# Advanced-Vision-and-Learning-Lab/sparse-view-3dgs-pack

Hardware: AMD Instinct MI355X
Metric: train-step views/s (fwd+bwd) @1M Gaussians 1080p (higher is better)
Workload: dtype f32

## Files before the change

### sparse-view-3dgs-pack_amd/csrc/gs_api.hip

```cpp
#include <stdio.h>
#include <stdlib.h>
#include <string.h>
#include <math.h>

#include "gs_common.h"
#include "gs_tilecull.h"
#include "gs_prof.h"

static int check_args(const GsView* v, const GsGaussians* g) {
  if (!v || !g) return GS_E_NULL;
  if (g->P < 0 || v->image_width <= 0 || v->image_height <= 0) return GS_E_SHAPE;
  if (g->P == 0) return GS_OK;
  if (!g->means3D || !g->opacities || !v->viewmatrix || !v->projmatrix || !v->bg) return GS_E_NULL;
  if ((g->shs == nullptr) == (g->colors_precomp == nullptr)) return GS_E_SHAPE;
  const bool has_sr = g->scales != nullptr && g->rotations != nullptr;
  const bool any_sr = g->scales != nullptr || g->rotations != nullptr;
  if ((!has_sr && g->cov3D_precomp == nullptr) || (any_sr && g->cov3D_precomp != nullptr)) return GS_E_SHAPE;
  if (g->shs && (g->M < (v->sh_degree + 1) * (v->sh_degree + 1) || !v->campos)) return GS_E_SHAPE;
  if (v->sh_degree < 0 || v->sh_degree > 3) return GS_E_SHAPE;
  if (g->shs_rest && (!g->shs || g->M < 2)) return GS_E_SHAPE;
  if (v->image_width > 65535 * TILE_X || v->image_height > 65535 * TILE_Y) return GS_E_UNSUPPORTED;
  return GS_OK;
}

static bool reached_marking() {
  static const bool on = [] { const char* e = getenv("GS_REACHED_SPLIT"); return !(e && atoi(e) == 0); }();
  return on;
}
static inline bool step_uses_reached(const GsStepState* st) {
  return st && st->reached_split && !st->rows_override && !st->grad_out[0];
}

static inline void tile_grid(const GsView* v, int& gx, int& gy) {
  gx = (v->image_width + TILE_X - 1) / TILE_X;
  gy = (v->image_height + TILE_Y - 1) / TILE_Y;
}

struct RegionLayout {
  uint32_t* count;
  uint2* bucket;
  uint32_t* point_list;
  uint32_t cap;
  int rg_x, rg_y;
};
static int region_layout(const GsView* v, const GsScratch* sc, RegionLayout& rl) {
// ... 236 lines not shown

  if (!sc->binned) {
    rc = forward_bin_stage(v, sc, gv, iv, bv, P, gx, gy, s);
    if (rc) return rc;
  }
  {
    GS_PROF(ST_RENDER_FWD, s);
    launch_render_fwd_wave(iv.ranges, bv.vals[0], W, H, gx, gy, gv.splat, v->bg, iv.final_T, iv.n_contrib, iv.tile_work,
                           sc->tile_order_hint, sc->tile_depth_limit, iv.tile_stop_depth, &gv.hdr->trunc_failed, out_color,
                           out_invdepth, out_extra, fsgs, v->tile_cull ? 0 : 1, s, reached_marking() ? gv.reached : nullptr,
                           &gv.hdr->pad[HDR_REACHED]);
  }
  if (!sc->defer_tile_order) {
    GS_PROF(ST_TILE_ORDER, s);
    launch_tile_order(iv.tile_work, iv.tile_order, (int)T, sc->tile_order_out, iv.tile_stop_depth, sc->tile_depth_limit_out, gx, gy,
                      gv.hdr, s, sc->tile_depth_limit_slack, sc->status_host, sc->step_tag);
  }
  GS_LAUNCH_CHECK(s, v->debug);
  return GS_OK;
}

int gs_backward(const GsView* v, const GsGaussians* g, const int32_t* radii, const GsScratch* sc,
                int64_t num_rendered, const float* dL_dcolor, const float* dL_dinvdepth, const GsGrads* grads,
                void* workspace, size_t workspace_bytes, void* stream) {
  return gs_backward_x(v, g, radii, sc, num_rendered, dL_dcolor, dL_dinvdepth, nullptr, grads, workspace, workspace_bytes,
                       stream);
}

static int backward_impl(const GsView* v, const GsGaussians* g, const int32_t* radii, const GsScratch* sc,
                         int64_t num_rendered, const float* dL_dcolor, const float* dL_dinvdepth, const float* dL_dextra,
                         int fsgs, const GsGrads* grads, void* workspace, size_t workspace_bytes, void* stream,
// ... 32 lines not shown
  a.P = g->P;
  a.D = v->sh_degree;
  a.M = g->M;
  a.means3D = g->means3D;
  a.radii = radii;
  a.shs = g->shs;
  a.shs_rest = g->shs_rest;
  a.scales = g->scales;
  a.rotations = g->rotations;
  a.opacities = g->opacities;
  a.raw_activations = g->raw_activations;
  a.skip_uninstanced = 0;
  a.tiles_touched = gv.tiles_touched;
  a.reached = nullptr;
  a.reached_flag = nullptr;
  a.colors_precomp = g->colors_precomp;
  a.scale_modifier = v->scale_modifier;
  a.cov3D = g->cov3D_precomp ? g->cov3D_precomp : gv.cov3D;
  a.viewmatrix = v->viewmatrix;
  a.projmatrix = v->projmatrix;
  a.campos = v->campos;
  a.focal_y = v->image_height / (2.0f * v->tanfovy);
  a.focal_x = v->image_width / (2.0f * v->tanfovx);
  a.tan_fovx = v->tanfovx;
  a.tan_fovy = v->tanfovy;
  a.antialiasing = v->antialiasing;
  a.has_invdepth = depth_mode;
  a.has_extra = g->extra_channel != nullptr;
  a.extra_raw = a.extra_gain = nullptr;
  a.gain_partials = nullptr;
// ... 88 lines not shown
  }
  if (num_rendered > 0 && !given_rows) {
    {
      GS_PROF(ST_RENDER_BWD, s);
      launch_render_bwd_wave(iv.ranges, bv.vals[0], W, H, gx, gy, gv.splat, v->bg, iv.final_T, iv.n_contrib, iv.tile_work,
                             iv.tile_order, dL_dcolor, dL_dinvdepth, dL_dextra, rows, fsgs, s);
    }
    GS_LAUNCH_CHECK(s, v->debug);
  }
  PreprocessBwdArgs a = preprocess_bwd_args(v, g, radii, gv, fsgs ? 2 : (dL_dinvdepth != nullptr ? 1 : 0), rows, recs, grads);
  a.skip_uninstanced = (v->tile_cull || (step && step->phase == 2)) ? 1 : 0;
  a.clean_rows = rows_clean != 0;
  if (step_uses_reached(step)) {
    a.reached = gv.reached;
    a.reached_flag = &gv.hdr->pad[HDR_REACHED];
  }
  if (step && step->extra) {
    float* gp = reinterpret_cast<float*>((char*)workspace + gs_align((size_t)P * GR_ROW_BYTES) + gs_align((size_t)P * GC_REC_BYTES));
    a.extra_raw = step->extra;
    a.extra_gain = step->gain;
    a.gain_partials = gp;
    sa.gain_partials = gp;
  }
  {
    GS_PROF(ST_CHAIN, s);
    launch_chain(a, step ? gv.hdr : nullptr, s);
  }
  if (step) {
    GS_PROF(ST_BWD_STEP, s);
    sa.hdr = gv.hdr;
// ... 407 lines not shown
  hdr->pad[0] = gs_status_check(t, hdr->num_rendered, hdr->overflow, hdr->trunc_failed);
}

int gs_forward_tile_order(const GsView* v, const GsScratch* sc, void* stream) {
  if (!v || !sc || !sc->geom || !sc->img) return GS_E_NULL;
  const int W = v->image_width, H = v->image_height;
  if (W <= 0 || H <= 0) return GS_E_SHAPE;
  int gx, gy;
  tile_grid(v, gx, gy);
  const size_t T = (size_t)gx * gy, N = (size_t)W * H;
  if (sc->img_bytes < img_bytes(N, T) || sc->geom_bytes < sizeof(GeomHeader)) return GS_E_SCRATCH;
  hipStream_t s = (hipStream_t)stream;
  ImgView iv = img_view(sc->img, N, T);
  GS_PROF(ST_TILE_ORDER, s);
  launch_tile_order(iv.tile_work, iv.tile_order, (int)T, sc->tile_order_out, iv.tile_stop_depth, sc->tile_depth_limit_out, gx, gy,
                    (const GeomHeader*)sc->geom, s, sc->tile_depth_limit_slack, sc->status_host, sc->step_tag);
  GS_LAUNCH_CHECK(s, v->debug);
  return GS_OK;
}

int gs_forward_status(const GsScratch* sc, uint32_t* out, void* stream) {
  if (!sc || !sc->geom || !out) return GS_E_NULL;
  if (sc->geom_bytes < sizeof(GeomHeader)) return GS_E_SCRATCH;
  hipStream_t s = (hipStream_t)stream;
  size_t bytes = 16;
  if (sc->step_tag) {
    (void)hipGetLastError();
    hipLaunchKernelGGL(status_tag_kernel, dim3(1), dim3(1), 0, s, (GeomHeader*)sc->geom, sc->step_tag);
    GS_LAUNCH_CHECK(s, 0);
    bytes = 48;
  }
// ... 96 lines not shown
```

### sparse-view-3dgs-pack_amd/csrc/gs_backward_math.h

```cpp
#pragma once
#include "gs_common.h"
#include "gs_math.h"

struct ShRegsB {
  float f[48];
  __host__ __device__ __forceinline__ V3 operator()(int k) const { return {f[3 * k], f[3 * k + 1], f[3 * k + 2]}; }
};

#define SH_LDS_ROW 19
struct ShSink {
  float* p;
  bool basis_only;
  float* rest = nullptr;
  __host__ __device__ __forceinline__ void rgb(V3 g) const {
    if (basis_only) {
      p[16] = g.x;
      p[17] = g.y;
      p[18] = g.z;
    }
  }
  __host__ __device__ __forceinline__ void set(int k, float basis, V3 g) const {
    if (basis_only) {
      p[k] = basis;
    } else {
// ... 210 lines not shown
}


struct GeomBack {
  V3 dmean;
  float dmean2D_x, dmean2D_y;
  float dcov[6];
  float dop, dextra;
  V3 dcolor;
  V3 dscale;
  float dq[4];
};
GS_DEV void chain_from_row(const PreprocessBwdArgs& a, int idx, const gs_row_t* row, float* rec) {
  const double2* gr = reinterpret_cast<const double2*>(row);
  const double2 g0 = gr[0], g1 = gr[1], g2 = gr[2], g3 = gr[3], g4 = gr[4], g5 = gr[5];
  const V3 mean = {a.means3D[3 * idx], a.means3D[3 * idx + 1], a.means3D[3 * idx + 2]};
  SymD Sg;
  RotD R = {};
  D3 s = {0.0, 0.0, 0.0};
  V4 rq = {1.f, 0.f, 0.f, 0.f};
  if (a.scales) {
    const V3 scl = load_scales(a.scales, idx, a.raw_activations);
    rq = load_rotation(a.rotations, idx, a.raw_activations);
    const double mod = a.scale_modifier;
    s = {mod * scl.x, mod * scl.y, mod * scl.z};
    R = quat_to_Rd(rq);
    Sg = sigma_from_scale_rot(s, R);
  } else {
    const float2* cv = reinterpret_cast<const float2*>(a.cov3D + 6 * (size_t)idx);
    const float2 v0 = cv[0], v1 = cv[1], v2 = cv[2];
// ... 8 lines not shown
    const float* vm = a.viewmatrix;
    const float zc = vm[2] * mean.x + vm[6] * mean.y + vm[10] * mean.z + vm[14];
    const float gd = (float)g4.y;
    dmean = dmean + V3{(vm[2] - vm[3] * zc) * gd, (vm[6] - vm[7] * zc) * gd, (vm[10] - vm[11] * zc) * gd};
  }
  float c[7] = {0.f, 0.f, 0.f, 0.f, 0.f, 0.f, 0.f};
  if (a.scales) {
    V3 dscale;
    cov3d_backward(cb.G, s, R, rq, dscale, c + 3);
    c[0] = dscale.x; c[1] = dscale.y; c[2] = dscale.z;
  } else {
    c[0] = (float)cb.G.xx; c[1] = (float)(2.0 * cb.G.xy); c[2] = (float)(2.0 * cb.G.xz);
    c[3] = (float)cb.G.yy; c[4] = (float)(2.0 * cb.G.yz); c[5] = (float)cb.G.zz;
  }
  float4* o = reinterpret_cast<float4*>(rec);
  o[0] = make_float4((float)g0.x, (float)g0.y, dmean.x, dmean.y);
  o[1] = make_float4(dmean.z, cb.dop, c[0], c[1]);
  o[2] = make_float4(c[2], c[3], c[4], c[5]);
  o[3] = make_float4(c[6], (float)g3.x, (float)g3.y, (float)g4.x);
  o[4] = make_float4((float)g5.x, 0.f, 0.f, 0.f);
}

GS_DEV void geometry_backward(const PreprocessBwdArgs& a, int idx, GeomBack& o) {
  const float4* rc = reinterpret_cast<const float4*>(a.grad_recs + (size_t)idx * GC_STRIDE);
  const float4 r0 = rc[0], r1 = rc[1], r2 = rc[2], r3 = rc[3];
  o.dmean2D_x = r0.x;
  o.dmean2D_y = r0.y;
  o.dop = r1.y;
  o.dcolor = {r3.y, r3.z, r3.w};
  o.dextra = a.has_extra ? a.grad_recs[(size_t)idx * GC_STRIDE + GC_EXTRA] : 0.f;
  const V3 mean = {a.means3D[3 * idx], a.means3D[3 * idx + 1], a.means3D[3 * idx + 2]};
  o.dmean = V3{r0.z, r0.w, r1.x} + projection_backward(mean, a.projmatrix, o.dmean2D_x, o.dmean2D_y);
  o.dscale = {0.f, 0.f, 0.f};
  o.dq[0] = o.dq[1] = o.dq[2] = o.dq[3] = 0.f;
  o.dcov[0] = o.dcov[1] = o.dcov[2] = o.dcov[3] = o.dcov[4] = o.dcov[5] = 0.f;
// ... 54 lines not shown
```

### sparse-view-3dgs-pack_amd/csrc/gs_common.h

```cpp
#pragma once
#include <hip/hip_runtime.h>
#include <stdint.h>

#include "../../include/gsplat.h"

#define GS_BLOCK 256
#define TILE_X GS_TILE_X
#define TILE_Y GS_TILE_Y

struct GeomHeader {
  uint32_t num_rendered;
  uint32_t overflow;
  uint32_t trunc_failed;
  uint32_t zero;
  uint32_t P;
  uint32_t sort_n;
  uint32_t n_ordered;
  uint32_t region_mode;
  uint32_t step_tag;
  uint32_t pad[55];
};
#define HDR_SIDE_CURSOR 1
#define HDR_LIMITED 2
#define HDR_REACHED 3
static_assert(sizeof(GeomHeader) == 256, "header is one 256-B block");

struct __attribute__((aligned(64))) Splat {
  float x, y;
  float depth;
  float invdepth;
  float cxx, cxy, cyy;
  float opacity;
  float r, g, b;
  float extra;
  uint32_t rect_min;
  uint32_t rect_max;
  uint32_t tiles;
  uint32_t clamped;
};
// ... 34 lines not shown
  b.vals[1] = (uint32_t*)p; p += gs_align(4 * cap);
  b.hist = (uint32_t*)p; p += gs_align(4 * hist_n);
  b.scan_tmp = (uint32_t*)p; p += gs_align(4 * RS_RADIX_MAX);
  return b;
}

struct GeomView {
  GeomHeader* hdr;
  Splat* splat;
  float* cov3D;
  uint32_t* tiles_touched;
  uint32_t* block_sums;
  uint32_t* sorted_sums;
  uint32_t* depth_keys;
  SortBufs gsort;
  uint8_t* reached;
};
static inline __host__ __device__ size_t geom_bytes(size_t P) {
  size_t nb = (P + GS_BLOCK - 1) / GS_BLOCK;
  return sizeof(GeomHeader) + gs_align(64 * P) + gs_align(24 * P) + 2 * gs_align(4 * P) + 2 * gs_align(4 * (nb + 1)) +
         sort_bytes(P) + gs_align(P);
}
static inline __host__ __device__ GeomView geom_view(void* buf, size_t P) {
  char* p = (char*)buf;
  size_t nb = (P + GS_BLOCK - 1) / GS_BLOCK;
  GeomView g;
  g.hdr = (GeomHeader*)p; p += sizeof(GeomHeader);
  g.splat = (Splat*)p; p += gs_align(64 * P);
  g.cov3D = (float*)p; p += gs_align(24 * P);
  g.tiles_touched = (uint32_t*)p; p += gs_align(4 * P);
  g.block_sums = (uint32_t*)p; p += gs_align(4 * (nb + 1));
  g.sorted_sums = (uint32_t*)p; p += gs_align(4 * (nb + 1));
  g.depth_keys = (uint32_t*)p; p += gs_align(4 * P);
  g.gsort = sort_view(p, P); p += sort_bytes(P);
  g.reached = (uint8_t*)p;
  return g;
}

#define RG_COUNT_STRIDE 32
struct ImgView {
  float* final_T;
  uint32_t* n_contrib;
  uint2* ranges;
  uint32_t* tile_work;
  uint32_t* tile_order;
  float* tile_stop_depth;
  uint32_t* region_count;
};
static inline __host__ __device__ size_t img_bytes(size_t N, size_t T) {
// ... 141 lines not shown
int launch_region_bin(const GeomView& g, const uint32_t* region_count, const uint2* region_bucket, uint32_t region_cap, int rg_x,
                      int rg_y, int grid_x, int grid_y, const float* tile_depth_limit, uint2* ranges, uint32_t* point_list,
                      int64_t capacity, hipStream_t s);
int launch_export_keys_region(const uint2* ranges, const uint32_t* point_list, const Splat* splat, int T, uint64_t* keys_sorted,
                              hipStream_t s);


int launch_render_fwd_wave(const uint2* ranges, const uint32_t* point_list, int W, int H, int grid_x, int grid_y,
                           const Splat* splat, const float* bg, float* final_T, uint32_t* n_contrib, uint32_t* tile_work,
                           const uint32_t* order_hint, const float* depth_limit, float* stop_depth, uint32_t* trunc_failed,
                           float* out_color, float* out_invdepth, float* out_extra, int fsgs, int cull, hipStream_t s,
                           uint8_t* reached = nullptr, uint32_t* reached_flag = nullptr);
int launch_export_stop_depth(const float* stop_depth, float* out, int grid_x, int grid_y, hipStream_t s);
int launch_tile_order(const uint32_t* tile_work, uint32_t* tile_order, int T, uint32_t* order_out, const float* stop_depth,
                      float* limit_out, int grid_x, int grid_y, const GeomHeader* hdr, hipStream_t s,
                      const float* slack_dev = nullptr, uint32_t* status_host = nullptr, const uint32_t* step_tag = nullptr);
int launch_zero_rows(gs_row_t* rows, size_t P, const uint32_t* tiles_touched, hipStream_t s);
int launch_render_bwd_wave(const uint2* ranges, const uint32_t* point_list, int W, int H, int grid_x, int grid_y,
                           const Splat* splat, const float* bg, const float* final_T, const uint32_t* n_contrib,
                           const uint32_t* tile_work, const uint32_t* tile_order, const float* dL_dpix,
                           const float* dL_dinvdepth, const float* dL_dextra, gs_row_t* grad_rows, int fsgs, hipStream_t s);

int launch_depth_fwd(const uint2* ranges, const uint32_t* point_list, int W, int H, int grid_x, int grid_y, const Splat* splat,
                     float* final_T, uint32_t* n_contrib, uint32_t* tile_work, float* stop_depth, float* out_depth,
                     float* out_alpha, int cull, hipStream_t s);
int launch_depth_bwd(const uint2* ranges, const uint32_t* point_list, int W, int H, int grid_x, int grid_y, const Splat* splat,
                     const float* final_T, const uint32_t* n_contrib, const uint32_t* tile_work, const uint32_t* tile_order,
                     const float* dL_ddepth, const float* dL_dalpha, gs_row_t* grad_rows, int grad_flags, hipStream_t s);
struct DepthPointArgs {
  int P;
  const float* means3D;
// ... 43 lines not shown
  float focal_x, focal_y, tan_fovx, tan_fovy;
  int antialiasing;
  int has_invdepth;
  int has_extra;
  const float* extra_raw;
  const float* extra_gain;
  float* gain_partials;
  int raw_activations;
  int skip_uninstanced;
  const gs_row_t* grad_rows;
  float* grad_recs;
  int clean_rows;
  const uint32_t* tiles_touched;
  const uint8_t* reached;
  const uint32_t* reached_flag;
  const Splat* splat;
  GsGrads out;
};
static inline __device__ bool gs_use_reached(const PreprocessBwdArgs& a) {
  return a.reached != nullptr && a.reached_flag[0] != 0u;
}
static inline __device__ bool gs_instanced(const PreprocessBwdArgs& a, bool use_reached, int idx) {
  return use_reached ? a.reached[idx] != 0 : a.tiles_touched[idx] != 0u;
}
int launch_chain(const PreprocessBwdArgs& a, const GeomHeader* hdr, hipStream_t s);
int launch_preprocess_bwd(const PreprocessBwdArgs& a, hipStream_t s, float* dsh_rest_out = nullptr);
struct StepArgs {
  GsStepState st;
  float lr_bc1[6];
  float inv_sqrt_bc2[5];
// ... 8 lines not shown
```

### sparse-view-3dgs-pack_amd/csrc/gs_preprocess.hip

```cpp
#include "gs_common.h"
#include "gs_tilecull.h"
#include "gs_math.h"

template <typename SH>
GS_DEV V3 color_from_sh(int deg, V3 pos, V3 campos, const SH& sh, uint32_t& clamped) {
  V3 dir = pos - campos;
  dir = dir / length3(dir);
  V3 result = SH_C0 * sh(0);
  if (deg > 0) {
    float x = dir.x, y = dir.y, z = dir.z;
    result = result - SH_C1 * y * sh(1) + SH_C1 * z * sh(2) - SH_C1 * x * sh(3);
    if (deg > 1) {
      float xx = x * x, yy = y * y, zz = z * z;
      float xy = x * y, yz = y * z, xz = x * z;
      result = result + SH_C2_0 * xy * sh(4) + SH_C2_1 * yz * sh(5) + SH_C2_2 * (2.0f * zz - xx - yy) * sh(6) +
               SH_C2_3 * xz * sh(7) + SH_C2_4 * (xx - yy) * sh(8);
      if (deg > 2) {
        result = result + SH_C3_0 * y * (3.0f * xx - yy) * sh(9) + SH_C3_1 * xy * z * sh(10) +
                 SH_C3_2 * y * (4.0f * zz - xx - yy) * sh(11) + SH_C3_3 * z * (2.0f * zz - 3.0f * xx - 3.0f * yy) * sh(12) +
                 SH_C3_4 * x * (4.0f * zz - xx - yy) * sh(13) + SH_C3_5 * z * (xx - yy) * sh(14) +
                 SH_C3_6 * x * (xx - 3.0f * yy) * sh(15);
      }
    }
  }
// ... 82 lines not shown
  float op_in = a.opacities[lidx];
  V3 p_orig = {a.means3D[3 * (size_t)lidx], a.means3D[3 * (size_t)lidx + 1], a.means3D[3 * (size_t)lidx + 2]};
  V3 sc_in = {sc_p[0], sc_p[1], sc_p[2]};
  V4 rq_in = {rq_p[0], rq_p[1], rq_p[2], rq_p[3]};
  if (lds_floats) {
    const float* src = a.tile_depth_limit + (GS_LIMIT_TILES_IN_LDS ? 0 : T);
    for (int i = threadIdx.x; i < lds_floats; i += GS_BLOCK) s_limit[i] = src[i];
    __syncthreads();
  }
  asm volatile("" : "+v"(op_in), "+v"(sc_in.x), "+v"(sc_in.y), "+v"(sc_in.z), "+v"(rq_in.x), "+v"(rq_in.y), "+v"(rq_in.z),
               "+v"(rq_in.w));
  const GsLdsFloatPtr lds_seg = (GsLdsFloatPtr)s_limit + (GS_LIMIT_TILES_IN_LDS ? T : 0);
  if (idx == 0) {
    g.hdr->pad[HDR_LIMITED] = a.tile_depth_limit ? 1u : 0u;
    g.hdr->pad[HDR_REACHED] = 0u;
  }
  const int segs_x = (int)depth_limit_segs_x((uint32_t)a.grid_x);
  auto region_bound = [&](int rx, int ry) {
    float bound = -__builtin_inff();
#pragma unroll
    for (int k = 0; k < RG_TILES; k++) {
      const int ty = min(ry * RG_TILES + k, a.grid_y - 1);
      const float v = lds_floats ? lds_seg[ty * segs_x + rx] : a.tile_depth_limit[(size_t)T + ty * segs_x + rx];
      bound = fmaxf(bound, v);
    }
    return bound;
  };
  Splat sp;
  sp.x = sp.y = sp.depth = sp.invdepth = 0.f;
  sp.cxx = sp.cxy = sp.cyy = sp.opacity = 0.f;
// ... 427 lines not shown
```

### sparse-view-3dgs-pack_amd/csrc/gs_preprocess_bwd.hip

```cpp
#include "gs_common.h"
#include "gs_math.h"
#include "gs_backward_math.h"

#define CHAIN_PER_WAVE 256
__global__ void __launch_bounds__(64, 3) chain_kernel(PreprocessBwdArgs a, const GeomHeader* hdr) {
  __shared__ int s_list[CHAIN_PER_WAVE];
  const int lane = threadIdx.x;
  const int base = blockIdx.x * CHAIN_PER_WAVE;
  bool has[CHAIN_PER_WAVE / 64];
  const bool use_reached = gs_use_reached(a);
  const bool list_reached = use_reached && !a.gain_partials;
#pragma unroll
  for (int k = 0; k < CHAIN_PER_WAVE / 64; k++) {
    const int idx = base + k * 64 + lane;
    has[k] = idx < a.P && a.radii[idx] > 0 && !(a.skip_uninstanced && !gs_instanced(a, list_reached, idx));
  }
  int n = 0;
#pragma unroll
  for (int k = 0; k < CHAIN_PER_WAVE / 64; k++) {
    const unsigned long long m = __ballot(has[k]);
    if (has[k]) s_list[n + __popcll(m & ((1ull << lane) - 1ull))] = base + k * 64 + lane;
    n += __popcll(m);
  }
  __syncthreads();
  const bool failed = hdr && (hdr->overflow | hdr->trunc_failed) != 0u;
  float gc = 1.0f, dgain = 0.f;
  bool gain_free = false;
  if (a.gain_partials) {
    const float gain = *a.extra_gain;
    gc = clamp_gain(gain);
    gain_free = gain >= 0.1f && gain <= 10.0f;
  }
  for (int j = lane; j < n; j += 64) {
    const int idx = s_list[j];
    if (use_reached && !list_reached && a.reached[idx] == 0) continue;
    gs_row_t* row = const_cast<gs_row_t*>(a.grad_rows) + (size_t)idx * GR_STRIDE;
    float* rec = a.grad_recs + (size_t)idx * GC_STRIDE;
    if (!failed) {
      chain_from_row(a, idx, row, rec);
      if (a.gain_partials) {
        const float dextra = rec[GC_EXTRA];
        if (gain_free) dgain += dextra * (1.0f / (1.0f + expf(-a.extra_raw[idx])));
        rec[GC_EXTRA] = dextra * gc;
      }
    }
    if (a.clean_rows) {
      float4* w = reinterpret_cast<float4*>(row);
      w[0] = w[1] = w[2] = w[3] = w[4] = w[5] = make_float4(0.f, 0.f, 0.f, 0.f);
    }
  }
  if (a.gain_partials) {
#pragma unroll
    for (int off = 32; off >= 1; off >>= 1) dgain += __shfl_down(dgain, off, 64);
    if (lane == 0) a.gain_partials[blockIdx.x] = dgain;
  }
}
int launch_chain(const PreprocessBwdArgs& a, const GeomHeader* hdr, hipStream_t s) {
  hipLaunchKernelGGL(chain_kernel, dim3((a.P + CHAIN_PER_WAVE - 1) / CHAIN_PER_WAVE), dim3(64), 0, s, a, hdr);
  return 0;
}

template <int N, typename G>
__device__ __forceinline__ void grad_block(float* __restrict__ out, int first, int cnt, const G& grad) {
// ... 503 lines not shown
```

### sparse-view-3dgs-pack_amd/csrc/gs_render_fwd_wave.hip

```cpp
#include "gs_blend.h"
#include "gs_common.h"
#include "gs_tilecull.h"

#define WB 64

template <bool HAS_EXTRA, bool FSGS, bool CULL>
__global__ void __launch_bounds__(64) render_fwd_wave_kernel(const uint2* __restrict__ ranges,
                                                             const uint32_t* __restrict__ point_list, int W, int H,
                                                             int grid_x, const Splat* __restrict__ splat,
                                                             const float* __restrict__ bg, float* __restrict__ final_T,
                                                             uint32_t* __restrict__ n_contrib,
                                                             uint32_t* __restrict__ tile_work,
                                                             const uint32_t* __restrict__ order_hint,
                                                             const float* __restrict__ depth_limit,
                                                             float* __restrict__ stop_depth,
                                                             uint32_t* __restrict__ trunc_failed,
                                                             float* __restrict__ out_color,
                                                             float* __restrict__ out_invdepth,
                                                             float* __restrict__ out_extra,
                                                             uint8_t* __restrict__ reached,
                                                             uint32_t* __restrict__ reached_flag) {
  __shared__ float4 s_a[WB];
  __shared__ float4 s_c[WB];
  __shared__ float4 s_k[WB];
// ... 155 lines not shown
  if (fsgs) {
    if (cull) GS_FWD_WAVE(false, true, true); else GS_FWD_WAVE(false, true, false);
  } else if (out_extra) {
    if (cull) GS_FWD_WAVE(true, false, true); else GS_FWD_WAVE(true, false, false);
  } else {
    if (cull) GS_FWD_WAVE(false, false, true); else GS_FWD_WAVE(false, false, false);
  }
#undef GS_FWD_WAVE
  return 0;
}

#define TO_THREADS 1024
#define TO_BUCKETS 2048
__device__ __forceinline__ void stop_depth_bound_item(const float* __restrict__ stop, float* __restrict__ out, int grid_x,
                                                      int grid_y, int i, float slack = 1.0f);
__global__ void __launch_bounds__(TO_THREADS) tile_order_kernel(const uint32_t* __restrict__ tile_work,
                                                                uint32_t* __restrict__ tile_order, int T, int per_band,
                                                                uint32_t* __restrict__ order_out,
                                                                const float* __restrict__ stop_depth,
                                                                float* __restrict__ limit_out, int grid_x, int grid_y,
                                                                const GeomHeader* __restrict__ hdr,
                                                                const float* __restrict__ slack_dev,
                                                                uint32_t* status_host, const uint32_t* step_tag) {
  if (status_host && blockIdx.x == 0 && threadIdx.x == 0) {
    const uint32_t nr = hdr->num_rendered, ov = hdr->overflow, tf = hdr->trunc_failed;
    volatile uint32_t* out = status_host;
    out[0] = nr; out[1] = ov; out[2] = tf; out[3] = hdr->zero;
    if (step_tag) {
      const uint32_t t = *step_tag;
      out[9] = gs_status_check(t, nr, ov, tf);
      __threadfence_system();
      out[8] = t;
    }
    __threadfence_system();
  }
  if (hdr->overflow) order_out = nullptr;
  if (blockIdx.x >= 8) {
    const int i = (int)(blockIdx.x - 8) * TO_THREADS + (int)threadIdx.x;
    if (!hdr->overflow && i < (int)depth_limit_floats((uint32_t)grid_x, (uint32_t)grid_y))
      stop_depth_bound_item(stop_depth, limit_out, grid_x, grid_y, i, slack_dev ? fmaxf(*slack_dev, 1.0f) : 1.0f);
    return;
  }
  __shared__ uint32_t s_cnt[TO_BUCKETS];
  __shared__ uint32_t s_part[TO_THREADS / 64];
  __shared__ uint32_t s_max;
  const int tid = threadIdx.x;
  const int band = blockIdx.x;
  const int t_lo = band * per_band, t_hi = min(T, t_lo + per_band);
  uint32_t m = 0;
  for (int t = t_lo + tid; t < t_hi; t += TO_THREADS) m = max(m, tile_work[t]);
#pragma unroll
// ... 58 lines not shown
}
__global__ void __launch_bounds__(256) stop_depth_bounds_kernel(const float* __restrict__ stop, float* __restrict__ out,
                                                                int grid_x, int grid_y) {
  const int i = blockIdx.x * 256 + threadIdx.x;
  if (i < (int)depth_limit_floats((uint32_t)grid_x, (uint32_t)grid_y)) stop_depth_bound_item(stop, out, grid_x, grid_y, i);
}

int launch_export_stop_depth(const float* stop_depth, float* out, int grid_x, int grid_y, hipStream_t s) {
  const int n = (int)depth_limit_floats((uint32_t)grid_x, (uint32_t)grid_y);
  hipLaunchKernelGGL(stop_depth_bounds_kernel, dim3((n + 255) / 256), dim3(256), 0, s, stop_depth, out, grid_x, grid_y);
  return 0;
}

int launch_tile_order(const uint32_t* tile_work, uint32_t* tile_order, int T, uint32_t* order_out, const float* stop_depth,
                      float* limit_out, int grid_x, int grid_y, const GeomHeader* hdr, hipStream_t s, const float* slack_dev,
                      uint32_t* status_host, const uint32_t* step_tag) {
  const int extra = limit_out ? ((int)depth_limit_floats((uint32_t)grid_x, (uint32_t)grid_y) + TO_THREADS - 1) / TO_THREADS : 0;
  hipLaunchKernelGGL(tile_order_kernel, dim3(8 + extra), dim3(TO_THREADS), 0, s, tile_work, tile_order, T, (T + 7) / 8, order_out,
                     stop_depth, limit_out, grid_x, grid_y, hdr, slack_dev, status_host, step_tag);
  return 0;
}
```

### sparse-view-3dgs-pack_amd/gsplat_amd/raster.py

```python
import ctypes as C
import os

import torch

from .capi import GsGaussians, GsGrads, GsScratch, GsView

NUM_CHANNELS = 3
_DEPTH_ONLY = 2


def _ptr(t):
    if t is None or t.numel() == 0:
        return None
    return t.data_ptr()


def _prep(t, device):
    if t is None or t.numel() == 0:
        return None
    if t.dtype != torch.float32:
        t = t.float()
    if t.device != device:
        t = t.to(device)
    return t.contiguous()
# ... 326 lines not shown
        self.api.raw("region_coop")(int(bool(on)))

    scratch_fill = None
    output_fill = None
    KEYED_LIMITS = os.environ.get("GS_KEYED_LIMITS", "1") != "0"
    STATUS_IN_RENDER = True

    def _side_stream(self, device):
        side = self._side_streams.get(device.index)
        if side is None:
            side = self._side_streams[device.index] = torch.cuda.Stream(device=device)
        return side
    TWO_PHASE = os.environ.get("GS_TWO_PHASE_STEP", "1") != "0"
    TWO_PHASE_MIN_P = 100_000
    REACHED_SPLIT = os.environ.get("GS_REACHED_SPLIT", "1") != "0"

    def _two_phase(self, step, P):
        return self.TWO_PHASE and P >= self.TWO_PHASE_MIN_P and not step.grad_out[0]

    def _arms_side_launch(self, step, P):
        return self._two_phase(step, P) and not step.rows_override

    def launch_uninstanced_early(self):
        f = self._last
        if f is None or f.step is None or f.done is not None:
            return False
        f.done = self._launch_uninstanced(f.geom.device, f.view, f.g, f.radii, self._scratch(f.geom, f.img), f.step)
        return True

    def _structs(self, device, bg, means3D, sh, colors_precomp, opacities, scales, rotations, cov3D_precomp, viewmatrix,
                 projmatrix, campos, tanfovx, tanfovy, H, W, scale_modifier, degree, antialiasing, debug, extra=None, raw=False,
                 extra_gain=None, sh_rest=None):
        keep = []
        view = self._view(keep, device, bg, viewmatrix, projmatrix, campos, tanfovx, tanfovy, H, W, scale_modifier, degree,
                          False, antialiasing, debug)
        g = self._gauss(keep, device, means3D, sh, colors_precomp, opacities, scales, rotations, cov3D_precomp, extra, raw=raw,
                        extra_gain=extra_gain, sh_rest=sh_rest)
        return view, g, keep

    def _launch_uninstanced(self, device, view, g, radii, s, step):
        main = torch.cuda.current_stream(device)
        side = self._side_stream(device)
        side.wait_stream(main)
        step.reached_split = int(self.REACHED_SPLIT)
        self.api.call("step_uninstanced", C.byref(view), C.byref(g), radii.contiguous().data_ptr(), C.byref(s),
                      C.byref(step), C.c_void_p(side.cuda_stream))
        done = torch.cuda.Event()
        done.record(side)
        self.two_phase_launches += 1
        return done

    def rasterize_gaussians(self, bg, means3D, colors_precomp, opacities, scales, rotations, scale_modifier,
                            cov3D_precomp, viewmatrix, projmatrix, tanfovx, tanfovy, image_height, image_width,
                            sh, degree, campos, prefiltered, antialiasing, debug, extra=None, fsgs=False, extra_gain=None):
        if fsgs and (extra is not None or antialiasing):
            raise RuntimeError("the FSGS rasterizer generation has neither anti-aliasing nor a 4th channel")
        if means3D.ndim != 2 or means3D.shape[1] != 3:
            raise RuntimeError("means3D must have dimensions (num_points, 3)")
        self._check_device(means3D)
# ... 393 lines not shown
        return z

    def _backward_step_fsgs(self, step, view, g, radii, geom, binning, img, P, W, H, R, dL_dout_color, dL_ddepth, dL_dalpha):
        device = radii.device
        if step.phase != 0 or step.phase1_done:
            raise RuntimeError("the two-phase step (side launch of gs_step_uninstanced) is closed to the FSGS rasterizer "
                               "generation")
        if step.extra:
            raise RuntimeError("the FSGS rasterizer generation has no 4th channel to step")
        _, _, _, wsb = self.scratch_bytes(P, W, H, R)
        ws = self._rows_workspace(step, device, wsb)
        s = self._scratch(geom, img, binning, self._capacity_for(binning, P, W, H, R))
        last = self._last
        if last is not None:
            last.step = last.radii = last.img = last.done = None
        step.reached_split = int(self.REACHED_SPLIT)
        dL_ddepth, dL_dalpha = _prep(dL_ddepth, device), _prep(dL_dalpha, device)
        zeros = self._zero_image(device, H, W) if dL_ddepth is None or dL_dalpha is None else None
        try:
            self.api.call("backward_step_fsgs", C.byref(view), C.byref(g), radii.data_ptr(), C.byref(s), int(R),
                          dL_dout_color.data_ptr(), (dL_ddepth if dL_ddepth is not None else zeros).data_ptr(),
                          (dL_dalpha if dL_dalpha is not None else zeros).data_ptr(), C.byref(step), _ptr(ws), ws.numel(),
                          self._stream(device))
        except Exception:
            self.rows_epoch += 1
            raise
        if step.rows_clean:
            self._rows_ws[(device.index, wsb)][1] = True
        return (None,) * 8

    def _backward_step(self, step, f, view, g, radii, geom, binning, img, P, W, H, R, dL_dout_color, dL_dout_invdepth,
                       dL_dout_extra, fsgs=False):
        if fsgs:
            return self._backward_step_fsgs(step, view, g, radii, geom, binning, img, P, W, H, R, dL_dout_color,
                                            dL_dout_invdepth, dL_dout_extra)
        device = radii.device
        _, _, _, wsb = self.scratch_bytes(P, W, H, R)
        ws = self._rows_workspace(step, device, wsb)
        s = self._scratch(geom, img, binning, self._capacity_for(binning, P, W, H, R))
        done, last = None, self._last
        if last is not None:
            if last is f and last.step is step:
                done = last.done
            last.step = last.radii = last.img = last.done = None
        if done is None:
            step.reached_split = int(self.REACHED_SPLIT)
        if self._two_phase(step, P):
            if done is None:
                done = self._launch_uninstanced(device, view, g, radii, s, step)
            self._uninst_done = done
            step.phase = 2
            step.phase1_done = done.cuda_event
        try:
            if dL_dout_extra is not None:
                self.api.call("backward_step_x", C.byref(view), C.byref(g), radii.data_ptr(), C.byref(s), int(R),
                              dL_dout_color.data_ptr(), _ptr(dL_dout_invdepth), dL_dout_extra.data_ptr(), C.byref(step),
                              _ptr(ws), ws.numel(), self._stream(device))
            else:
                self.api.call("backward_step", C.byref(view), C.byref(g), radii.data_ptr(), C.byref(s), int(R),
                              dL_dout_color.data_ptr(), _ptr(dL_dout_invdepth), C.byref(step), _ptr(ws), ws.numel(),
                              self._stream(device))
# ... 124 lines not shown
        P = int(means3D.shape[0])
        present = torch.zeros((P,), dtype=torch.bool, device=device)
        if P != 0:
            m, vm, pm = (_prep(x, device) for x in (means3D, viewmatrix, projmatrix))
            self.api.call("mark_visible", P, m.data_ptr(), vm.data_ptr(), pm.data_ptr(), present.data_ptr(),
                          self._stream(device))
        return present

    def export_reached(self, P, geom):
        gb = self.scratch_bytes(P, 16, 16, 0)[0]
        off = gb - ((P + 255) // 256) * 256
        if geom.device.type == "cuda":
            torch.cuda.current_stream(geom.device).synchronize()
        return geom[off:off + P].clone()

    def export_state(self, P, W, H, R, geom, binning, img):
        device = geom.device
        cap = self._capacity_for(binning, P, W, H, R)
        s = self._scratch(geom, img, binning, cap)
        f32 = dict(dtype=torch.float32, device=device)
        T = ((W + 15) // 16) * ((H + 15) // 16)
        out = dict(
            depths=torch.zeros((P,), **f32), means2D=torch.zeros((P, 2), **f32), cov3D=torch.zeros((P, 6), **f32),
            conic_opacity=torch.zeros((P, 4), **f32), rgb=torch.zeros((P, 3), **f32),
            clamped=torch.zeros((P, 3), dtype=torch.uint8, device=device),
            tiles_touched=torch.zeros((P,), dtype=torch.int32, device=device),
            point_offsets=torch.zeros((P,), dtype=torch.int32, device=device),
            keys_sorted=torch.zeros((R,), dtype=torch.int64, device=device),
            point_list=torch.zeros((R,), dtype=torch.int32, device=device),
            final_T=torch.zeros((H, W), **f32), n_contrib=torch.zeros((H, W), dtype=torch.int32, device=device),
# ... 18 lines not shown
```

Baseline: 1261.

## Build compacted reached-Gaussian list in tile-order kernel and drive chain backward from it

Extra workgroups appended to the tile-order kernel compact the per-Gaussian reached flags into per-segment index lists with counts. The backward chain kernel then walks this compact list instead of scanning all P Gaussians with radii, instanced and reached checks, so it should launch less idle work when only a fraction were reached. In exchange the geometry scratch grows by about 4 bytes per Gaussian, the tile-order kernel does more work, and every chain wave runs a prefix scan over segment counts. It also pins the rec-store values in registers with empty asm statements.

```diff
diff --git a/sparse-view-3dgs-pack_amd/csrc/gs_api.hip b/sparse-view-3dgs-pack_amd/csrc/gs_api.hip
--- a/sparse-view-3dgs-pack_amd/csrc/gs_api.hip
+++ b/sparse-view-3dgs-pack_amd/csrc/gs_api.hip
@@ -28,7 +28,14 @@
   return on;
 }
 static inline bool step_uses_reached(const GsStepState* st) {
-  return st && st->reached_split && !st->rows_override && !st->grad_out[0];
+  return st && (st->reached_split & 1) && !st->rows_override && !st->grad_out[0];
+}
+static bool reached_listing() {
+  static const bool on = [] { const char* e = getenv("GS_REACHED_LIST"); return !(e && atoi(e) == 0); }();
+  return on && reached_marking();
+}
+static inline bool step_uses_reached_list(const GsStepState* st) {
+  return step_uses_reached(st) && !(st->reached_split & 2) && !st->extra && reached_listing();
 }
 
 static inline void tile_grid(const GsView* v, int& gx, int& gy) {
@@ -295,7 +302,8 @@
   if (!sc->defer_tile_order) {
     GS_PROF(ST_TILE_ORDER, s);
     launch_tile_order(iv.tile_work, iv.tile_order, (int)T, sc->tile_order_out, iv.tile_stop_depth, sc->tile_depth_limit_out, gx, gy,
-                      gv.hdr, s, sc->tile_depth_limit_slack, sc->status_host, sc->step_tag);
+                      gv.hdr, s, sc->tile_depth_limit_slack, sc->status_host, sc->step_tag, reached_listing() ? sc->geom : nullptr,
+                      sc->geom_bytes, P);
   }
   GS_LAUNCH_CHECK(s, v->debug);
   return GS_OK;
@@ -358,6 +366,7 @@
   a.tiles_touched = gv.tiles_touched;
   a.reached = nullptr;
   a.reached_flag = nullptr;
+  a.reached_list = a.reached_counts = a.reached_list_flag = nullptr;
   a.colors_precomp = g->colors_precomp;
   a.scale_modifier = v->scale_modifier;
   a.cov3D = g->cov3D_precomp ? g->cov3D_precomp : gv.cov3D;
@@ -476,6 +485,11 @@
   if (step_uses_reached(step)) {
     a.reached = gv.reached;
     a.reached_flag = &gv.hdr->pad[HDR_REACHED];
+  }
+  if (step_uses_reached_list(step) && sc->geom_bytes >= geom_bytes((size_t)P)) {
+    a.reached_list = gv.reached_list;
+    a.reached_counts = gv.reached_counts;
+    a.reached_list_flag = &gv.hdr->pad[HDR_REACHED_LIST];
   }
   if (step && step->extra) {
     float* gp = reinterpret_cast<float*>((char*)workspace + gs_align((size_t)P * GR_ROW_BYTES) + gs_align((size_t)P * GC_REC_BYTES));
@@ -913,7 +927,8 @@
   ImgView iv = img_view(sc->img, N, T);
   GS_PROF(ST_TILE_ORDER, s);
   launch_tile_order(iv.tile_work, iv.tile_order, (int)T, sc->tile_order_out, iv.tile_stop_depth, sc->tile_depth_limit_out, gx, gy,
-                    (const GeomHeader*)sc->geom, s, sc->tile_depth_limit_slack, sc->status_host, sc->step_tag);
+                    (const GeomHeader*)sc->geom, s, sc->tile_depth_limit_slack, sc->status_host, sc->step_tag,
+                    reached_listing() ? sc->geom : nullptr, sc->geom_bytes, -1);
   GS_LAUNCH_CHECK(s, v->debug);
   return GS_OK;
 }
diff --git a/sparse-view-3dgs-pack_amd/csrc/gs_backward_math.h b/sparse-view-3dgs-pack_amd/csrc/gs_backward_math.h
--- a/sparse-view-3dgs-pack_amd/csrc/gs_backward_math.h
+++ b/sparse-view-3dgs-pack_amd/csrc/gs_backward_math.h
@@ -248,6 +248,8 @@
 GS_DEV void chain_from_row(const PreprocessBwdArgs& a, int idx, const gs_row_t* row, float* rec) {
   const double2* gr = reinterpret_cast<const double2*>(row);
   const double2 g0 = gr[0], g1 = gr[1], g2 = gr[2], g3 = gr[3], g4 = gr[4], g5 = gr[5];
+  float p_mx = (float)g0.x, p_my = (float)g0.y, p_r = (float)g3.x, p_g = (float)g3.y, p_b = (float)g4.x, p_x = (float)g5.x;
+  asm volatile("" : "+v"(p_mx), "+v"(p_my), "+v"(p_r), "+v"(p_g), "+v"(p_b), "+v"(p_x));
   const V3 mean = {a.means3D[3 * idx], a.means3D[3 * idx + 1], a.means3D[3 * idx + 2]};
   SymD Sg;
   RotD R = {};
@@ -286,11 +288,11 @@
     c[3] = (float)cb.G.yy; c[4] = (float)(2.0 * cb.G.yz); c[5] = (float)cb.G.zz;
   }
   float4* o = reinterpret_cast<float4*>(rec);
-  o[0] = make_float4((float)g0.x, (float)g0.y, dmean.x, dmean.y);
+  o[0] = make_float4(p_mx, p_my, dmean.x, dmean.y);
   o[1] = make_float4(dmean.z, cb.dop, c[0], c[1]);
   o[2] = make_float4(c[2], c[3], c[4], c[5]);
-  o[3] = make_float4(c[6], (float)g3.x, (float)g3.y, (float)g4.x);
-  o[4] = make_float4((float)g5.x, 0.f, 0.f, 0.f);
+  o[3] = make_float4(c[6], p_r, p_g, p_b);
+  o[4] = make_float4(p_x, 0.f, 0.f, 0.f);
 }
 
 GS_DEV void geometry_backward(const PreprocessBwdArgs& a, int idx, GeomBack& o) {
diff --git a/sparse-view-3dgs-pack_amd/csrc/gs_common.h b/sparse-view-3dgs-pack_amd/csrc/gs_common.h
--- a/sparse-view-3dgs-pack_amd/csrc/gs_common.h
+++ b/sparse-view-3dgs-pack_amd/csrc/gs_common.h
@@ -23,6 +23,7 @@
 #define HDR_SIDE_CURSOR 1
 #define HDR_LIMITED 2
 #define HDR_REACHED 3
+#define HDR_REACHED_LIST 4
 static_assert(sizeof(GeomHeader) == 256, "header is one 256-B block");
 
 struct __attribute__((aligned(64))) Splat {
@@ -87,12 +88,16 @@
   uint32_t* sorted_sums;
   uint32_t* depth_keys;
   SortBufs gsort;
+  uint32_t* reached_list;
+  uint32_t* reached_counts;
   uint8_t* reached;
 };
+#define RL_SEG 65536
+static inline __host__ __device__ size_t reached_list_segments(size_t P) { return (P + RL_SEG - 1) / RL_SEG; }
 static inline __host__ __device__ size_t geom_bytes(size_t P) {
   size_t nb = (P + GS_BLOCK - 1) / GS_BLOCK;
   return sizeof(GeomHeader) + gs_align(64 * P) + gs_align(24 * P) + 2 * gs_align(4 * P) + 2 * gs_align(4 * (nb + 1)) +
-         sort_bytes(P) + gs_align(P);
+         sort_bytes(P) + gs_align(4 * P) + gs_align(4 * reached_list_segments(P)) + gs_align(P);
 }
 static inline __host__ __device__ GeomView geom_view(void* buf, size_t P) {
   char* p = (char*)buf;
@@ -106,6 +111,8 @@
   g.sorted_sums = (uint32_t*)p; p += gs_align(4 * (nb + 1));
   g.depth_keys = (uint32_t*)p; p += gs_align(4 * P);
   g.gsort = sort_view(p, P); p += sort_bytes(P);
+  g.reached_list = (uint32_t*)p; p += gs_align(4 * P);
+  g.reached_counts = (uint32_t*)p; p += gs_align(4 * reached_list_segments(P));
   g.reached = (uint8_t*)p;
   return g;
 }
@@ -277,7 +284,8 @@
 int launch_export_stop_depth(const float* stop_depth, float* out, int grid_x, int grid_y, hipStream_t s);
 int launch_tile_order(const uint32_t* tile_work, uint32_t* tile_order, int T, uint32_t* order_out, const float* stop_depth,
                       float* limit_out, int grid_x, int grid_y, const GeomHeader* hdr, hipStream_t s,
-                      const float* slack_dev = nullptr, uint32_t* status_host = nullptr, const uint32_t* step_tag = nullptr);
+                      const float* slack_dev = nullptr, uint32_t* status_host = nullptr, const uint32_t* step_tag = nullptr,
+                      void* list_geom = nullptr, size_t list_geom_bytes = 0, int64_t list_P = -1);
 int launch_zero_rows(gs_row_t* rows, size_t P, const uint32_t* tiles_touched, hipStream_t s);
 int launch_render_bwd_wave(const uint2* ranges, const uint32_t* point_list, int W, int H, int grid_x, int grid_y,
                            const Splat* splat, const float* bg, const float* final_T, const uint32_t* n_contrib,
@@ -351,6 +359,9 @@
   const uint32_t* tiles_touched;
   const uint8_t* reached;
   const uint32_t* reached_flag;
+  const uint32_t* reached_list;
+  const uint32_t* reached_counts;
+  const uint32_t* reached_list_flag;
   const Splat* splat;
   GsGrads out;
 };
diff --git a/sparse-view-3dgs-pack_amd/csrc/gs_preprocess.hip b/sparse-view-3dgs-pack_amd/csrc/gs_preprocess.hip
--- a/sparse-view-3dgs-pack_amd/csrc/gs_preprocess.hip
+++ b/sparse-view-3dgs-pack_amd/csrc/gs_preprocess.hip
@@ -120,6 +120,7 @@
   if (idx == 0) {
     g.hdr->pad[HDR_LIMITED] = a.tile_depth_limit ? 1u : 0u;
     g.hdr->pad[HDR_REACHED] = 0u;
+    g.hdr->pad[HDR_REACHED_LIST] = 0u;
   }
   const int segs_x = (int)depth_limit_segs_x((uint32_t)a.grid_x);
   auto region_bound = [&](int rx, int ry) {
diff --git a/sparse-view-3dgs-pack_amd/csrc/gs_preprocess_bwd.hip b/sparse-view-3dgs-pack_amd/csrc/gs_preprocess_bwd.hip
--- a/sparse-view-3dgs-pack_amd/csrc/gs_preprocess_bwd.hip
+++ b/sparse-view-3dgs-pack_amd/csrc/gs_preprocess_bwd.hip
@@ -3,26 +3,64 @@
 #include "gs_backward_math.h"
 
 #define CHAIN_PER_WAVE 256
+__device__ __forceinline__ int chain_list_entry(const PreprocessBwdArgs& a, uint32_t* s_incl, uint32_t e0, uint32_t& total) {
+  const int lane = threadIdx.x;
+  const uint32_t nseg = (uint32_t)reached_list_segments((size_t)a.P);
+  const uint32_t e = e0 + (uint32_t)lane;
+  uint32_t carry = 0u, seg = 0u, off = 0u;
+  bool found = false;
+  for (uint32_t c = 0; c < nseg; c += 64u) {
+    uint32_t incl = (c + lane < nseg) ? a.reached_counts[c + lane] : 0u;
+#pragma unroll
+    for (int o = 1; o < 64; o <<= 1) {
+      const uint32_t up = (uint32_t)__shfl_up((int)incl, o, 64);
+      if (lane >= o) incl += up;
+    }
+    incl += carry;
+    s_incl[lane] = incl;
+    __syncthreads();
+    const uint32_t after = s_incl[63];
+    if (!found && e < after) {
+      int lo = 0;
+#pragma unroll
+      for (int step = 32; step >= 1; step >>= 1)
+        if (s_incl[lo + step - 1] <= e) lo += step;
+      seg = c + (uint32_t)lo;
+      off = e - (lo ? s_incl[lo - 1] : carry);
+      found = true;
+    }
+    carry = after;
+    __syncthreads();
+  }
+  total = carry;
+  const size_t slot = (size_t)seg * RL_SEG + off;
+  if (!found || slot >= (size_t)a.P) return -1;
+  const uint32_t idx = a.reached_list[slot];
+  return (idx < (uint32_t)a.P && a.radii[idx] > 0) ? (int)idx : -1;
+}
 __global__ void __launch_bounds__(64, 3) chain_kernel(PreprocessBwdArgs a, const GeomHeader* hdr) {
   __shared__ int s_list[CHAIN_PER_WAVE];
   const int lane = threadIdx.x;
   const int base = blockIdx.x * CHAIN_PER_WAVE;
   bool has[CHAIN_PER_WAVE / 64];
   const bool use_reached = gs_use_reached(a);
+  const bool list_mode = a.reached_list && use_reached && a.skip_uninstanced && !a.gain_partials && a.reached_list_flag[0] != 0u;
   const bool list_reached = use_reached && !a.gain_partials;
-#pragma unroll
-  for (int k = 0; k < CHAIN_PER_WAVE / 64; k++) {
-    const int idx = base + k * 64 + lane;
-    has[k] = idx < a.P && a.radii[idx] > 0 && !(a.skip_uninstanced && !gs_instanced(a, list_reached, idx));
-  }
   int n = 0;
-#pragma unroll
-  for (int k = 0; k < CHAIN_PER_WAVE / 64; k++) {
-    const unsigned long long m = __ballot(has[k]);
-    if (has[k]) s_list[n + __popcll(m & ((1ull << lane) - 1ull))] = base + k * 64 + lane;
-    n += __popcll(m);
-  }
-  __syncthreads();
+  if (!list_mode) {
+#pragma unroll
+    for (int k = 0; k < CHAIN_PER_WAVE / 64; k++) {
+      const int idx = base + k * 64 + lane;
+      has[k] = idx < a.P && a.radii[idx] > 0 && !(a.skip_uninstanced && !gs_instanced(a, list_reached, idx));
+    }
+#pragma unroll
+    for (int k = 0; k < CHAIN_PER_WAVE / 64; k++) {
+      const unsigned long long m = __ballot(has[k]);
+      if (has[k]) s_list[n + __popcll(m & ((1ull << lane) - 1ull))] = base + k * 64 + lane;
+      n += __popcll(m);
+    }
+    __syncthreads();
+  }
   const bool failed = hdr && (hdr->overflow | hdr->trunc_failed) != 0u;
   float gc = 1.0f, dgain = 0.f;
   bool gain_free = false;
@@ -31,22 +69,36 @@
     gc = clamp_gain(gain);
     gain_free = gain >= 0.1f && gain <= 10.0f;
   }
-  for (int j = lane; j < n; j += 64) {
-    const int idx = s_list[j];
-    if (use_reached && !list_reached && a.reached[idx] == 0) continue;
-    gs_row_t* row = const_cast<gs_row_t*>(a.grad_rows) + (size_t)idx * GR_STRIDE;
-    float* rec = a.grad_recs + (size_t)idx * GC_STRIDE;
-    if (!failed) {
-      chain_from_row(a, idx, row, rec);
-      if (a.gain_partials) {
-        const float dextra = rec[GC_EXTRA];
-        if (gain_free) dgain += dextra * (1.0f / (1.0f + expf(-a.extra_raw[idx])));
-        rec[GC_EXTRA] = dextra * gc;
-      }
-    }
-    if (a.clean_rows) {
-      float4* w = reinterpret_cast<float4*>(row);
-      w[0] = w[1] = w[2] = w[3] = w[4] = w[5] = make_float4(0.f, 0.f, 0.f, 0.f);
+  for (uint32_t r = 0;; r++) {
+    int idx = -1;
+    if (list_mode) {
+      const uint32_t e0 = (blockIdx.x + r * gridDim.x) * 64u;
+      uint32_t total;
+      idx = chain_list_entry(a, reinterpret_cast<uint32_t*>(s_list), e0, total);
+      if (e0 >= total) break;
+    } else {
+      const int j = (int)r * 64 + lane;
+      if ((int)r * 64 >= n) break;
+      if (j < n) idx = s_list[j];
+      if (idx >= 0 && use_reached && !list_reached && a.reached[idx] == 0) idx = -1;
+    }
+    if (idx >= 0) {
+      gs_row_t* row = const_cast<gs_row_t*>(a.grad_rows) + (size_t)idx * GR_STRIDE;
+      float* rec = a.grad_recs + (size_t)idx * GC_STRIDE;
+      if (!failed) {
+        chain_from_row(a, idx, row, rec);
+        if (a.gain_partials) {
+          const float dextra = rec[GC_EXTRA];
+          if (gain_free) dgain += dextra * (1.0f / (1.0f + expf(-a.extra_raw[idx])));
+          rec[GC_EXTRA] = dextra * gc;
+        }
+      }
+      if (a.clean_rows) {
+        int idx2 = idx;
+        asm volatile("" : "+v"(idx2));
+        float4* w = reinterpret_cast<float4*>(const_cast<gs_row_t*>(a.grad_rows) + (size_t)idx2 * GR_STRIDE);
+        w[0] = w[1] = w[2] = w[3] = w[4] = w[5] = make_float4(0.f, 0.f, 0.f, 0.f);
+      }
     }
   }
   if (a.gain_partials) {
diff --git a/sparse-view-3dgs-pack_amd/csrc/gs_render_fwd_wave.hip b/sparse-view-3dgs-pack_amd/csrc/gs_render_fwd_wave.hip
--- a/sparse-view-3dgs-pack_amd/csrc/gs_render_fwd_wave.hip
+++ b/sparse-view-3dgs-pack_amd/csrc/gs_render_fwd_wave.hip
@@ -193,6 +193,60 @@
 #define TO_BUCKETS 2048
 __device__ __forceinline__ void stop_depth_bound_item(const float* __restrict__ stop, float* __restrict__ out, int grid_x,
                                                       int grid_y, int i, float slack = 1.0f);
+static_assert(RL_SEG == TO_THREADS * 64, "a thread of the segment's workgroup owns 64 flags");
+__device__ __forceinline__ void reached_list_segment(void* geom, size_t geom_have, uint32_t seg) {
+  __shared__ uint32_t s_wtot[TO_THREADS / 64];
+  GeomHeader* hdr = reinterpret_cast<GeomHeader*>(geom);
+  const uint32_t P = hdr->P;
+  if (hdr->pad[HDR_REACHED] == 0u || P == 0u || geom_bytes((size_t)P) > geom_have) return;
+  if ((size_t)seg * RL_SEG >= (size_t)P) return;
+  const GeomView g = geom_view(geom, (size_t)P);
+  const int tid = threadIdx.x, lane = tid & 63, wave = tid >> 6;
+  const uint32_t seg_row0 = seg * (uint32_t)RL_SEG;
+  const uint32_t wave_row0 = seg_row0 + (uint32_t)wave * 4096u;
+  const uint32_t row0 = wave_row0 + (uint32_t)lane * 64u;
+  unsigned long long m = 0ull;
+#pragma unroll
+  for (int q = 0; q < 4; q++) {
+    const uint32_t b = row0 + 16u * q;
+    if (b < P) {
+      const uint4 v = *reinterpret_cast<const uint4*>(g.reached + b);
+      const uint32_t w[4] = {v.x, v.y, v.z, v.w};
+#pragma unroll
+      for (int k = 0; k < 4; k++)
+#pragma unroll
+        for (int j = 0; j < 4; j++)
+          if ((w[k] >> (8 * j)) & 0xFFu) m |= 1ull << (16 * q + 4 * k + j);
+    }
+  }
+  if (row0 >= P) m = 0ull;
+  else if (P - row0 < 64u) m &= (1ull << (P - row0)) - 1ull;
+  const uint32_t cnt = (uint32_t)__popcll(m);
+  uint32_t wsum = cnt;
+#pragma unroll
+  for (int off = 32; off >= 1; off >>= 1) wsum += (uint32_t)__shfl_xor((int)wsum, off, 64);
+  if (lane == 0) s_wtot[wave] = wsum;
+  __syncthreads();
+  uint32_t pos = 0, total = 0;
+  for (int w = 0; w < TO_THREADS / 64; w++) {
+    const uint32_t t = s_wtot[w];
+    if (w < wave) pos += t;
+    total += t;
+  }
+  if (tid == 0) {
+    g.reached_counts[seg] = total;
+    if (seg == 0u) hdr->pad[HDR_REACHED_LIST] = 1u;
+  }
+  if (wsum == 0u) return;
+  uint32_t* out = g.reached_list + seg_row0;
+  const uint32_t m_lo = (uint32_t)m, m_hi = (uint32_t)(m >> 32);
+  for (int i = 0; i < 64; i++) {
+    const unsigned long long mi = ((unsigned long long)(uint32_t)__shfl((int)m_hi, i, 64) << 32) | (uint32_t)__shfl((int)m_lo, i, 64);
+    if (mi == 0ull) continue;
+    if ((mi >> lane) & 1ull) out[pos + (uint32_t)__popcll(mi & ((1ull << lane) - 1ull))] = wave_row0 + 64u * i + (uint32_t)lane;
+    pos += (uint32_t)__popcll(mi);
+  }
+}
 __global__ void __launch_bounds__(TO_THREADS) tile_order_kernel(const uint32_t* __restrict__ tile_work,
                                                                 uint32_t* __restrict__ tile_order, int T, int per_band,
                                                                 uint32_t* __restrict__ order_out,
@@ -200,7 +254,8 @@
                                                                 float* __restrict__ limit_out, int grid_x, int grid_y,
                                                                 const GeomHeader* __restrict__ hdr,
                                                                 const float* __restrict__ slack_dev,
-                                                                uint32_t* status_host, const uint32_t* step_tag) {
+                                                                uint32_t* status_host, const uint32_t* step_tag,
+                                                                void* list_geom, size_t list_geom_bytes, int list_first) {
   if (status_host && blockIdx.x == 0 && threadIdx.x == 0) {
     const uint32_t nr = hdr->num_rendered, ov = hdr->overflow, tf = hdr->trunc_failed;
     volatile uint32_t* out = status_host;
@@ -214,6 +269,10 @@
     __threadfence_system();
   }
   if (hdr->overflow) order_out = nullptr;
+  if (list_geom && (int)blockIdx.x >= list_first) {
+    reached_list_segment(list_geom, list_geom_bytes, (uint32_t)((int)blockIdx.x - list_first));
+    return;
+  }
   if (blockIdx.x >= 8) {
     const int i = (int)(blockIdx.x - 8) * TO_THREADS + (int)threadIdx.x;
     if (!hdr->overflow && i < (int)depth_limit_floats((uint32_t)grid_x, (uint32_t)grid_y))
@@ -302,9 +361,15 @@
 
 int launch_tile_order(const uint32_t* tile_work, uint32_t* tile_order, int T, uint32_t* order_out, const float* stop_depth,
                       float* limit_out, int grid_x, int grid_y, const GeomHeader* hdr, hipStream_t s, const float* slack_dev,
-                      uint32_t* status_host, const uint32_t* step_tag) {
+                      uint32_t* status_host, const uint32_t* step_tag, void* list_geom, size_t list_geom_bytes, int64_t list_P) {
   const int extra = limit_out ? ((int)depth_limit_floats((uint32_t)grid_x, (uint32_t)grid_y) + TO_THREADS - 1) / TO_THREADS : 0;
-  hipLaunchKernelGGL(tile_order_kernel, dim3(8 + extra), dim3(TO_THREADS), 0, s, tile_work, tile_order, T, (T + 7) / 8, order_out,
-                     stop_depth, limit_out, grid_x, grid_y, hdr, slack_dev, status_host, step_tag);
+  int segs = 0;
+  if (list_geom) {
+    const size_t p_hi = list_P >= 0 ? (size_t)list_P : list_geom_bytes / 113;
+    segs = (int)reached_list_segments(p_hi);
+  }
+  hipLaunchKernelGGL(tile_order_kernel, dim3(8 + extra + segs), dim3(TO_THREADS), 0, s, tile_work, tile_order, T, (T + 7) / 8,
+                     order_out, stop_depth, limit_out, grid_x, grid_y, hdr, slack_dev, status_host, step_tag,
+                     segs > 0 ? list_geom : nullptr, list_geom_bytes, 8 + extra);
   return 0;
 }
diff --git a/sparse-view-3dgs-pack_amd/gsplat_amd/raster.py b/sparse-view-3dgs-pack_amd/gsplat_amd/raster.py
--- a/sparse-view-3dgs-pack_amd/gsplat_amd/raster.py
+++ b/sparse-view-3dgs-pack_amd/gsplat_amd/raster.py
@@ -364,6 +364,10 @@
     TWO_PHASE = os.environ.get("GS_TWO_PHASE_STEP", "1") != "0"
     TWO_PHASE_MIN_P = 100_000
     REACHED_SPLIT = os.environ.get("GS_REACHED_SPLIT", "1") != "0"
+    REACHED_LIST = os.environ.get("GS_REACHED_LIST", "1") != "0"
+
+    def _reached_split_word(self):
+        return (1 | (0 if self.REACHED_LIST else 2)) if self.REACHED_SPLIT else 0
 
     def _two_phase(self, step, P):
         return self.TWO_PHASE and P >= self.TWO_PHASE_MIN_P and not step.grad_out[0]
@@ -392,7 +396,7 @@
         main = torch.cuda.current_stream(device)
         side = self._side_stream(device)
         side.wait_stream(main)
-        step.reached_split = int(self.REACHED_SPLIT)
+        step.reached_split = self._reached_split_word()
         self.api.call("step_uninstanced", C.byref(view), C.byref(g), radii.contiguous().data_ptr(), C.byref(s),
                       C.byref(step), C.c_void_p(side.cuda_stream))
         done = torch.cuda.Event()
@@ -816,7 +820,7 @@
         last = self._last
         if last is not None:
             last.step = last.radii = last.img = last.done = None
-        step.reached_split = int(self.REACHED_SPLIT)
+        step.reached_split = self._reached_split_word()
         dL_ddepth, dL_dalpha = _prep(dL_ddepth, device), _prep(dL_dalpha, device)
         zeros = self._zero_image(device, H, W) if dL_ddepth is None or dL_dalpha is None else None
         try:
@@ -846,7 +850,7 @@
                 done = last.done
             last.step = last.radii = last.img = last.done = None
         if done is None:
-            step.reached_split = int(self.REACHED_SPLIT)
+            step.reached_split = self._reached_split_word()
         if self._two_phase(step, P):
             if done is None:
                 done = self._launch_uninstanced(device, view, g, radii, s, step)
@@ -1001,6 +1005,21 @@
             torch.cuda.current_stream(geom.device).synchronize()
         return geom[off:off + P].clone()
 
+    def export_reached_list(self, P, geom):
+        gb = self.scratch_bytes(P, 16, 16, 0)[0]
+        al = lambda n: ((n + 255) // 256) * 256
+        nseg = (P + 65535) // 65536
+        off_flags = gb - al(P)
+        off_counts = off_flags - al(4 * nseg)
+        off_list = off_counts - al(4 * P)
+        if geom.device.type == "cuda":
+            torch.cuda.current_stream(geom.device).synchronize()
+        built = int(geom[4 * 13:4 * 14].clone().view(torch.int32)[0])
+        counts = geom[off_counts:off_counts + 4 * nseg].clone().view(torch.int32).to(torch.int64)
+        words = geom[off_list:off_list + 4 * P].clone().view(torch.int32).to(torch.int64)
+        entries = [words[s * 65536:s * 65536 + int(counts[s])] if built else words[:0] for s in range(nseg)]
+        return built, counts, entries
+
     def export_state(self, P, W, H, R, geom, binning, img):
         device = geom.device
         cap = self._capacity_for(binning, P, W, H, R)
```

Measured after the change: 1277, median of 6. +1.3%, better.
